# GANtastic3/MaskCycleGAN-VC

Measured on AMD Instinct MI355X. Metric: train iters/s (full G+D step), 80x64 mel bs=1, higher is better.
Workload: dtype f32

## Files before the change

include/mcvc.h:

```cpp
#ifndef MCVC_H
#define MCVC_H

#ifdef __cplusplus
extern "C" {
#endif

#define MCVC_ABI_VERSION 3
#define MCVC_GEN_NPARAMS 110
#define MCVC_DISC_NPARAMS 20
#define MCVC_N_MEL 80

int mcvc_version(void);

int mcvc_set_deterministic(int on);
int mcvc_get_deterministic(void);
int mcvc_set_precise(int on);
int mcvc_get_precise(void);
int mcvc_set_trunk_persistent(int on);

int mcvc_twin_begin(void);
int mcvc_twin_switch(void);
int mcvc_twin_end(void);
int mcvc_twin_launches(void);

// ... 155 lines not shown

int mcvc_ms_max_fft(void);
int mcvc_ms_launches(void);
int mcvc_ms_table_init(int n_fft, float* table_host);
int mcvc_ms_power(const float* cep, long long n_frames, int K, const int* offs_dev, int n_utts, const int* offs_host, int n_fft, const float* table,
                  float* power, float* mean, float* var, void* stream);
int mcvc_ms_mean_log(const float* values, int n, long long R, float floor, float* out, void* stream);
int mcvc_ms_distance(const float* a, const float* b, int K, int n_bins, int n_used, float* per_dim, float* total, void* stream);

long long mcvc_conv2d_pack_floats(int Cout, int Cin, int KH, int KW);
int mcvc_conv2d_forward(const float* x, const float* w, const float* bias, float* y, float* wpack,
                        float* slabs, int max_slabs, int N, int Cin, int H, int W, int Cout, int KH, int KW,
                        int stride, int pad_h, int pad_w, int pixel_shuffle, void* stream);
int mcvc_conv2d_dgrad(const float* dy, const float* w, float* dx, float* wpack, float* slabs, int max_slabs,
                      int N, int Cin, int H, int W, int Cout, int KH, int KW, int stride, int pad_h, int pad_w,
                      void* stream);
long long mcvc_conv2d_wgrad_slab_floats(int N, int Cin, int H, int W, int Cout, int KH, int KW, int stride, int pad_h, int pad_w);
int mcvc_conv2d_wgrad(const float* x, const float* dy, float* dw, float* slabs, long long slab_floats, int N, int Cin, int H, int W,
                      int Cout, int KH, int KW, int stride, int pad_h, int pad_w, void* stream);
long long mcvc_layer_packed_floats(int Cin, int Cout, int branches, int KH, int KW, int stride, int pad_h, int pad_w);
long long mcvc_layer_scratch_floats(int N, int H, int W, int Cin, int Cout, int branches, int KH, int KW, int stride, int pad_h, int pad_w);
int mcvc_layer_pack(const float* w0, const float* b0, const float* w1, const float* b1, float* packed, int Cin, int Cout, int branches,
                    int KH, int KW, int stride, int pad_h, int pad_w, void* stream);
int mcvc_layer_forward(const float* x, const float* packed, const float* w0, const float* w1, float* y, float* scratch,
                       long long scratch_floats, int N, int H, int W, int Cin, int Cout, int branches, int KH, int KW, int stride,
                       int pad_h, int pad_w, int scheme, int pixel_shuffle, void* stream);
int mcvc_layer_dgrad(const float* dy, const float* packed, const float* w0, const float* w1, float* dx, float* scratch,
                     long long scratch_floats, int N, int H, int W, int Cin, int Cout, int branches, int KH, int KW, int stride,
                     int pad_h, int pad_w, int scheme, void* stream);
int mcvc_layer_wgrad(const float* x, const float* dy, float* dw0, float* dw1, float* scratch, long long scratch_floats, int N, int H,
                     int W, int Cin, int Cout, int branches, int KH, int KW, int stride, int pad_h, int pad_w, int scheme, void* stream);
int mcvc_layer_wgrad_flags(const float* x, const float* dy, float* dw0, float* dw1, float* scratch, long long scratch_floats, int N, int H,
                           int W, int Cin, int Cout, int branches, int KH, int KW, int stride, int pad_h, int pad_w, int scheme, int flags,
                           void* stream);
int mcvc_trunk_layer_backward(const float* dy, const float* conv_out, const float* stats, const float* gamma, const float* beta,
                              const float* gamma_gate, const float* beta_gate, const float* w, const float* w_gate, const float* x_in,
                              float* dx, float* dconv, float* dgamma, float* dbeta, float* dgamma_gate, float* dbeta_gate, float* dw,
                              float* dw_gate, float* wpack, int B, int Cin, int T4, int Cout, int KW, void* stream);

int mcvc_instnorm_act_forward(float* x, const float* gamma, const float* beta, const float* gamma_gate,
                              const float* beta_gate, const float* residual, float* y, float* stats,
                              int N, int C, int H, int W, int act, void* stream);
int mcvc_instnorm_act_backward(const float* x, const float* gamma, const float* beta, const float* gamma_gate,
                               const float* beta_gate, const float* stats, float* dy, float* dx,
                               float* dgamma, float* dbeta, float* dgamma_gate, float* dbeta_gate,
                               int N, int C, int H, int W, int act, void* stream);

int mcvc_trunk_layer_forward(const float* x, const float* w, const float* bias, const float* gamma, const float* beta, const float* w_gate,
                             const float* bias_gate, const float* gamma_gate, const float* beta_gate, const float* residual, float* conv_out,
                             float* stats, float* y, int B, int Cin, int T4, int Cout, int KW, void* stream);

int mcvc_batched_gemm(const float* a, const float* b, float* c, int nbatch, int M, int N, int K, int lda, int ldb, int ldc,
                      long long a_stride, long long b_stride, long long c_stride, void* stream);

int mcvc_bias_grad(const float* dy, float* db, int N, int C, int P, void* stream);
int mcvc_act_forward(float* x, float* y, int N, int C, int P, int act, void* stream);
int mcvc_act_backward(const float* x, float* dy, float* dx, int N, int C, int P, int act, void* stream);
int mcvc_fif_input(const float* x, const float* mask, float* xin, int N, int P, void* stream);
int mcvc_fif_input_grad(const float* dxin, const float* mask, float* dx, int N, int P, int accumulate, void* stream);

int mcvc_trace_enable(int on);
int mcvc_trace_kinds(void);
const char* mcvc_trace_kind_name(int kind);
int mcvc_trace_collect(double* out);
int mcvc_trace_collect_raw(double* out, int max_records);

#ifdef __cplusplus
}
#endif
#endif
```

maskcyclegan-vc_amd/csrc/net.hip:

```cpp
#include "mcvc_common.h"
#include "twin.h"
#include "pack.h"
#include "packforms.h"
#include "misc.h"
#include "trunk.h"
#include "wino.h"
#include "wino4.h"
#include "sgemm.h"
#include "sampler.h"
#include "audio.h"
#include "vocoder.h"
#include "griffinlim.h"
#include "melinv.h"
#include "dtw.h"
#include "ms.h"
#include "f0.h"
#include "../../include/mcvc.h"
#include <string.h>
#include <algorithm>
#include <array>
#include <tuple>
#include <map>
#include <mutex>
#include <vector>
// ... 2723 lines not shown
    } else rc = mcvc_trunk_launch(a, ks, s);
    if (rc || !x_in || !dw) return rc;
    if (KW != 3 || !mcvc_wgrad_smallk_batch_applies(B, T4)) return MCVC_ERR_INVALID;
    SmallKJob jobs[2];
    int nj = 0;
    jobs[nj++] = SmallKJob{x_in, dconv, dw, Cin, Cout, 0, 0};
    if (glu && dw_gate) jobs[nj++] = SmallKJob{x_in, dconv + (long long)Cout * B * T4, dw_gate, Cin, Cout, 0, 0};
    return mcvc_wgrad_smallk_batch_launch(jobs, nj, B, T4, s);
}

int mcvc_instnorm_act_forward(float* x, const float* gamma, const float* beta, const float* gamma_gate, const float* beta_gate,
                              const float* residual, float* y, float* stats, int N, int C, int H, int W, int act, void* stream)
{
    Exec ex{}; ex.s = (hipStream_t)stream;
    NormP np{}; np.g[0] = gamma; np.b[0] = beta; np.g[1] = gamma_gate; np.b[1] = beta_gate;
    const int Cx = (act == ACT_GLU) ? 2 * C : C;
    norm_fwd(ex, x, (long long)Cx * H * W, (long long)H * W, 0, 1, np, stats, y, (long long)C * H * W, (long long)H * W, W, residual, N, C, H, W, act);
    return ex.err;
}

int mcvc_instnorm_act_backward(const float* x, const float* gamma, const float* beta, const float* gamma_gate, const float* beta_gate,
                               const float* stats, float* dy, float* dx, float* dgamma, float* dbeta, float* dgamma_gate, float* dbeta_gate,
                               int N, int C, int H, int W, int act, void* stream)
{
    Exec ex{}; ex.s = (hipStream_t)stream;
    NormP np{}; np.g[0] = gamma; np.b[0] = beta; np.g[1] = gamma_gate; np.b[1] = beta_gate;
    np.dg[0] = dgamma; np.db[0] = dbeta; np.dg[1] = dgamma_gate; np.db[1] = dbeta_gate;
    const int Cx = (act == ACT_GLU) ? 2 * C : C;
    norm_bwd(ex, x, (long long)Cx * H * W, (long long)H * W, np, stats, dy, (long long)C * H * W, (long long)H * W, W, 0, 1,
             dx, (long long)Cx * H * W, (long long)H * W, W, 0, N, C, H, W, act);
    return ex.err;
}

int mcvc_trunk_layer_forward(const float* x, const float* w, const float* bias, const float* gamma, const float* beta, const float* w_gate,
                             const float* bias_gate, const float* gamma_gate, const float* beta_gate, const float* residual, float* conv_out,
                             float* stats, float* y, int B, int Cin, int T4, int Cout, int KW, void* stream)
{
    if (!x || !w || !bias || !gamma || !beta || !conv_out || !stats || !y) return MCVC_ERR_INVALID;
    const int mode = w_gate ? TRUNK_IN_GLU : TRUNK_IN;
    if (!mcvc_trunk_applies(Cin, KW, Cout, B, T4, mode, 1)) return MCVC_ERR_INVALID;
    TrunkArgs a{};
    a.a0 = w; a.bias0 = bias; a.gamma0 = gamma; a.beta0 = beta;
    a.a1 = w_gate; a.bias1 = bias_gate; a.gamma1 = gamma_gate; a.beta1 = beta_gate;
    a.x = x; a.x_sc = (long long)B * T4; a.x_sb = T4;
    a.Cin = Cin; a.KW = KW; a.K = Cin * KW; a.M = Cout; a.Mtot = w_gate ? 2 * Cout : Cout; a.B = B; a.T4 = T4; a.N = B * T4;
    a.conv_out = conv_out; a.c_sc = (long long)B * T4; a.c_sb = T4;
    a.stats = stats; a.y = y; a.res = residual; a.y_sn = T4; a.y_sc = (long long)B * T4; a.eps = kInEps; a.mode = mode;
    return mcvc_trunk_launch(a, 1, (hipStream_t)stream);
}

int mcvc_batched_gemm(const float* a, const float* b, float* c, int nbatch, int M, int N, int K, int lda, int ldb, int ldc,
                      long long a_stride, long long b_stride, long long c_stride, void* stream)
{
    if (!a || !b || !c || nbatch < 1) return MCVC_ERR_INVALID;
    WinoGemmArgs ga{};
    ga.a = a; ga.a_xi = a_stride; ga.lda = lda; ga.b = b; ga.b_xi = b_stride; ga.ldb = ldb; ga.c = c; ga.c_xi = c_stride; ga.ldc = ldc;
    ga.M = M; ga.N = N; ga.K = K; ga.nxi = nbatch;
    return mcvc_wino_gemm_launch(ga, (hipStream_t)stream);
}

int mcvc_bias_grad(const float* dy, float* db, int N, int C, int P, void* stream)
{
    return mcvc_bias_grad_launch(dy, (long long)C * P, (long long)P, N, C, P, db, (hipStream_t)stream);
}

int mcvc_act_forward(float* x, float* y, int N, int C, int P, int act, void* stream)
{
    Exec ex{}; ex.s = (hipStream_t)stream;
    act_fwd(ex, x, 0, 1, y, N, C, P, act);
    return ex.err;
}

int mcvc_act_backward(const float* x, float* dy, float* dx, int N, int C, int P, int act, void* stream)
{
    Exec ex{}; ex.s = (hipStream_t)stream;
    act_bwd(ex, x, dy, 0, 1, dx, N, C, P, act);
    return ex.err;
}

int mcvc_fif_input(const float* x, const float* mask, float* xin, int N, int P, void* stream)
{
    return mcvc_prep_input_launch(x, mask, xin, N, P, (hipStream_t)stream);
}

int mcvc_fif_input_grad(const float* dxin, const float* mask, float* dx, int N, int P, int accumulate, void* stream)
{
    return mcvc_mask_grad_launch(dxin, nullptr, 0, 1, mask, dx, N, P, 2, accumulate, (hipStream_t)stream);
}

}
```

maskcyclegan-vc_amd/csrc/wino.h:

```cpp
#pragma once
#include <hip/hip_runtime.h>

struct WinoXformArgs {
    const float* x; long long x_sb, x_sc; int x_sh;
    float* v;
    int N, C, H, W;
    int TH, TW, NT;
    int NTp;
    int pad;
};

struct WinoOutArgs {
    const float* m;
    const float* bias;
    float* y; long long y_sb, y_sc; int y_sh;
    int N, Cout, OH, OW, TH, TW, NT, NTp;
    int shuffle, YH, YW;
    int accumulate;
};

int mcvc_wino_input_launch(const WinoXformArgs& a, hipStream_t s);
struct NormArgs;
bool mcvc_norm_fwd_wino_applies(const NormArgs& a, const WinoOutArgs& w, int pts);
int mcvc_norm_fwd_wino_launch(const NormArgs& a, const WinoOutArgs& w, int pts, hipStream_t s);
// ... 10 lines not shown
static __device__ __forceinline__ void wino_weight_core(const float* g, float* dst, int co, int ci, int ld, long long xi_stride, int co_off, int dgrad)
{
    float gg[5][5];
#pragma unroll
    for (int k = 0; k < 5; ++k)
#pragma unroll
        for (int l = 0; l < 5; ++l) gg[k][l] = dgrad ? g[(4 - k) * 5 + (4 - l)] : g[k * 5 + l];
    auto grow = [](const float v[5], float o[6]) {
        const float s_even = v[0] + v[2] + v[4], s_odd = v[1] + v[3];
        o[0] = 0.25f * v[0];
        o[1] = -(s_even + s_odd) * (1.0f / 6.0f);
        o[2] = -(s_even - s_odd) * (1.0f / 6.0f);
        const float e2 = v[0] * (1.0f / 24.0f) + v[2] * (1.0f / 6.0f) + v[4] * (2.0f / 3.0f);
        const float o2 = v[1] * (1.0f / 12.0f) + v[3] * (1.0f / 3.0f);
        o[3] = e2 + o2;
        o[4] = e2 - o2;
        o[5] = v[4];
    };
    float t[5][6];
#pragma unroll
    for (int k = 0; k < 5; ++k) grow(gg[k], t[k]);
    const long long row = dgrad ? (co_off + co) : ci;
    const long long col = dgrad ? ci : (co_off + co);
    float* d0 = dst + row * ld + col;
#pragma unroll
    for (int b = 0; b < 6; ++b) {
        float colv[5], o[6];
#pragma unroll
        for (int k = 0; k < 5; ++k) colv[k] = t[k][b];
        grow(colv, o);
#pragma unroll
        for (int aa = 0; aa < 6; ++aa) d0[(long long)(aa * 6 + b) * xi_stride] = o[aa];
    }
}
static __device__ __forceinline__ void wino_weight_tile(const float* w, float* dst, int Cout, int Cin, int ld, long long xi_stride, int co_off, int dgrad, int bx, int by)
{
    const int a_idx = bx * 256 + threadIdx.x;
    const int b_idx = by;
    const int co = dgrad ? b_idx : a_idx, ci = dgrad ? a_idx : b_idx;
    if (co >= Cout || ci >= Cin) return;
    wino_weight_core(w + ((long long)co * Cin + ci) * 25, dst, co, ci, ld, xi_stride, co_off, dgrad);
}


struct WinoGemmArgs {
    const float* a; long long a_xi; int lda;
    const float* b; long long b_xi; int ldb;
    float* c; long long c_xi; int ldc;
    int M, N, K;
    int nxi;
    int nt, mt;
    int mgroup;
};
int mcvc_wino_gemm_launch(const WinoGemmArgs& a, hipStream_t s);

template <int P>
static __device__ __forceinline__ void wino_g3(float v0, float v1, float v2, float* o)
{
    if constexpr (P == 4) { o[0] = v0; o[1] = 0.5f * (v0 + v1 + v2); o[2] = 0.5f * (v0 - v1 + v2); o[3] = v2; }
    else {
        const float e = v0 + v2, e2 = v0 * (1.0f / 24.0f) + v2 * (1.0f / 6.0f);
        o[0] = 0.25f * v0; o[1] = -(e + v1) * (1.0f / 6.0f); o[2] = -(e - v1) * (1.0f / 6.0f);
        o[3] = e2 + v1 * (1.0f / 12.0f); o[4] = e2 - v1 * (1.0f / 12.0f); o[5] = v2;
    }
}

template <int P>
static __device__ __forceinline__ void wino3_weight_core_p(const float* g, float* dst, int co, int ci, int ld, long long xi_stride, int co_off)
{
    float gg[5][5];
#pragma unroll
    for (int k = 0; k < 25; ++k) gg[k / 5][k % 5] = g[k];
#pragma unroll
    for (int qh = 0; qh < 2; ++qh)
#pragma unroll
        for (int qw = 0; qw < 2; ++qw) {
            float t[3][P];
#pragma unroll
            for (int u = 0; u < 3; ++u) {
                const int kh = qh ? 5 - 2 * u : 4 - 2 * u;
                float r0 = 0.f, r1 = 0.f, r2 = 0.f;
                if (kh <= 4) {
                    if (qw) { r1 = gg[kh][3]; r2 = gg[kh][1]; }
                    else { r0 = gg[kh][4]; r1 = gg[kh][2]; r2 = gg[kh][0]; }
                }
                wino_g3<P>(r0, r1, r2, t[u]);
            }
            float* d0 = dst + (long long)(co_off + co) * ld + 4 * ci + 2 * qh + qw;
#pragma unroll
            for (int b = 0; b < P; ++b) {
                float o[P];
                wino_g3<P>(t[0][b], t[1][b], t[2][b], o);
#pragma unroll
                for (int aa = 0; aa < P; ++aa) d0[(long long)(aa * P + b) * xi_stride] = o[aa];
            }
        }
}

template <int P>
static __device__ __forceinline__ void wino3_weight_tile_p(const float* w, float* dst, int Cout, int Cin, int ld, long long xi_stride, int co_off, int bx, int by)
{
    const int ci = bx * 256 + threadIdx.x, co = by;
    if (co >= Cout || ci >= Cin) return;
    wino3_weight_core_p<P>(w + ((long long)co * Cin + ci) * 25, dst, co, ci, ld, xi_stride, co_off);
}

template <int P>
// ... 48 lines not shown
```

maskcyclegan-vc_amd/csrc/wino_kernels.hip:

```cpp
#include "mcvc_common.h"
#include "trace.h"
#include "launch.h"
#include "wino.h"

namespace {

__device__ __forceinline__ void bt6(const float d[6], float o[6])
{
    o[0] = 4.f * d[0] - 5.f * d[2] + d[4];
    o[1] = -4.f * (d[1] + d[2]) + d[3] + d[4];
    o[2] = 4.f * (d[1] - d[2]) - d[3] + d[4];
    o[3] = -2.f * d[1] - d[2] + 2.f * d[3] + d[4];
    o[4] = 2.f * d[1] - d[2] - 2.f * d[3] + d[4];
    o[5] = 4.f * d[1] - 5.f * d[3] + d[5];
}

__global__ void __launch_bounds__(256) wino_input_kernel(const Twin<WinoXformArgs> tw)
{
    const WinoXformArgs a = tw.v[blockIdx.z];
    const int tile = blockIdx.x * 256 + threadIdx.x;
    const int c = blockIdx.y;
    if (tile >= a.NT) return;
    const int per = a.TH * a.TW;
    const int n = tile / per, r = tile - n * per;
// ... 417 lines not shown

__global__ void __launch_bounds__(256) wino_output_kernel(const Twin<WinoOutArgs> tw)
{
    const WinoOutArgs a = tw.v[blockIdx.z];
    const int tile = blockIdx.x * 256 + threadIdx.x;
    const int co = blockIdx.y;
    if (tile >= a.NT) return;
    const int per = a.TH * a.TW;
    const int n = tile / per, r = tile - n * per;
    const int ty = r / a.TW, tx = r - ty * a.TW;
    const float* src = a.m + (long long)co * a.NTp + tile;
    const long long xs = (long long)a.Cout * a.NTp;
    float u[2][6];
#pragma unroll
    for (int b = 0; b < 6; ++b) {
        float col[6];
#pragma unroll
        for (int aa = 0; aa < 6; ++aa) col[aa] = src[(long long)(aa * 6 + b) * xs];
        at6(col, u[0][b], u[1][b]);
    }
    const float bias = a.bias ? a.bias[co] : 0.f;
    float* yn = a.y + (long long)n * a.y_sb;
#pragma unroll
    for (int i = 0; i < 2; ++i) {
        float o0, o1;
        at6(u[i], o0, o1);
        const float ov[2] = {o0 + bias, o1 + bias};
        const int oh = 2 * ty + i;
#pragma unroll
        for (int j = 0; j < 2; ++j) {
            const int ow = 2 * tx + j;
            if (oh >= a.OH || ow >= a.OW) continue;
            long long off;
            if (a.shuffle) {
                const int yh = 2 * oh + ((co >> 1) & 1), yw = 2 * ow + (co & 1);
                if (yh >= a.YH || yw >= a.YW) continue;
                off = (long long)(co >> 2) * a.y_sc + (long long)yh * a.y_sh + yw;
            } else {
                off = (long long)co * a.y_sc + (long long)oh * a.y_sh + ow;
            }
            if (a.accumulate) yn[off] += ov[j]; else yn[off] = ov[j];
        }
    }
}


constexpr int kGK = 16;
constexpr int kGStages = 4;
#ifndef MCVC_FOLDK
#define MCVC_FOLDK 32
#endif
constexpr int kFoldK = MCVC_FOLDK;
constexpr int kGA = kGK * 128;

__device__ __forceinline__ void wg_glds16(const float* g, float* l)
{
    __builtin_amdgcn_global_load_lds((const __attribute__((address_space(1))) void*)g,
                                     (__attribute__((address_space(3))) void*)l, 16, 0, 0);
}

template <int BN>
__global__ void __launch_bounds__(256, (BN == 64 ? 3 : 4)) wino_gemm_kernel(const Twin<WinoGemmArgs> tw)
{
    const WinoGemmArgs a = tw.v[blockIdx.z];
    constexpr int kGB = kGK * BN;
    constexpr int kGStage = kGA + kGB;
    constexpr int NACC = (BN == 64) ? 2 : 1;
    extern __shared__ __attribute__((aligned(16))) float smem[];
    const int tid = threadIdx.x, lane = tid & 63;
    const int wave = __builtin_amdgcn_readfirstlane(tid >> 6);
    const int l31 = lane & 31, half = lane >> 5;
    const int wm = (BN == 64) ? (wave >> 1) : wave, wn = (BN == 64) ? (wave & 1) : 0;
    int lid;
    {
        const int total = (int)gridDim.x, linear = (int)blockIdx.x;
        const int q = total >> 3, r = total & 7, xcd = linear & 7, k = linear >> 3;
        lid = (xcd < r ? xcd * (q + 1) : r * (q + 1) + (xcd - r) * q) + k;
    }
    const int n0 = (lid % a.nt) * BN; lid /= a.nt;
    const int m0 = (lid % a.mt) * 128;
    const int xi = lid / a.mt;
    const float* A = a.a + (long long)xi * a.a_xi + m0;
    const float* B = a.b + (long long)xi * a.b_xi + n0;
    const int fa0 = wave * 64 + lane, fa1 = fa0 + 256;
    const float* a_src0 = A + (long long)(fa0 >> 5) * a.lda + 4 * (fa0 & 31);
    const float* a_src1 = A + (long long)(fa1 >> 5) * a.lda + 4 * (fa1 & 31);
    const int bw = (BN == 64) ? wave : (wave & 1);
    const int fb = bw * 64 + lane;
    constexpr int F4R = BN / 4;
    int bcol = 4 * (fb % F4R);
    if (n0 + bcol > a.ldb - 4) bcol = a.ldb - 4 - n0;
    const float* b_src = B + (long long)(fb / F4R) * a.ldb + bcol;
    const long long a_step = (long long)kGK * a.lda, b_step = (long long)kGK * a.ldb;
    auto issue = [&](int stage_k, int buf) {
        float* base = smem + buf * kGStage;
        wg_glds16(a_src0 + stage_k * a_step, base + (wave * 64) * 4);
        wg_glds16(a_src1 + stage_k * a_step, base + (wave * 64 + 256) * 4);
        wg_glds16(b_src + stage_k * b_step, base + kGA + (bw * 64) * 4);
    };
    f32x16 acc[NACC], tot[NACC];
#pragma unroll
    for (int i = 0; i < NACC; ++i)
#pragma unroll
        for (int r = 0; r < 16; ++r) { acc[i][r] = 0.f; tot[i][r] = 0.f; }
    constexpr int kFoldSt = kFoldK / kGK;
    const int nst = a.K / kGK;
// ... 126 lines not shown
    const int b_lane = SA + half * BN + wn * (32 * NBN) + l31;
    for (int st = 0; st < nst; ++st) {
        const int newer = (nst - 1 - st) < (ST - 2) ? (nst - 1 - st) : (ST - 2);
        if (newer >= 2) wait_vm<2 * ND>(); else if (newer == 1) wait_vm<ND>(); else wait_vm<0>();
        __builtin_amdgcn_s_barrier();
        if (st + ST - 1 < nst) issue(st + ST - 1, (st + ST - 1) % ST);
        if (st != 0 && (st % kFoldSt) == 0) {
#pragma unroll
            for (int i = 0; i < NACC; ++i)
#pragma unroll
                for (int r = 0; r < 16; ++r) { tot[i][r] += acc[i][r]; acc[i][r] = 0.f; }
        }
        const float* sb = smem + (st % ST) * STAGE;
        float av[NBM], bv[NBN];
#pragma unroll
        for (int i = 0; i < NBM; ++i) av[i] = sb[a_lane + 32 * i];
#pragma unroll
        for (int j = 0; j < NBN; ++j) bv[j] = sb[b_lane + 32 * j];
#pragma unroll
        for (int p = 0; p < GK / 2; ++p) {
            const int q = (p + 1 < GK / 2) ? p + 1 : p;
            float na[NBM], nb[NBN];
#pragma unroll
            for (int i = 0; i < NBM; ++i) na[i] = sb[a_lane + q * 2 * BM + 32 * i];
#pragma unroll
            for (int j = 0; j < NBN; ++j) nb[j] = sb[b_lane + q * 2 * BN + 32 * j];
#pragma unroll
            for (int i = 0; i < NBM; ++i)
#pragma unroll
                for (int j = 0; j < NBN; ++j) acc[i * NBN + j] = __builtin_amdgcn_mfma_f32_32x32x2f32(av[i], bv[j], acc[i * NBN + j], 0, 0, 0);
            __builtin_amdgcn_sched_group_barrier(0x100, NBM + NBN, 0);
            __builtin_amdgcn_sched_group_barrier(0x008, NACC, 0);
#pragma unroll
            for (int i = 0; i < NBM; ++i) av[i] = na[i];
#pragma unroll
            for (int j = 0; j < NBN; ++j) bv[j] = nb[j];
        }
    }
    const long long ldc = a.ldc;
    const int Nv = a.N;
    float* Cb = a.c + (long long)xi * a.c_xi + (long long)(m0 + wm * (32 * NBM) + 4 * half) * ldc;
#pragma unroll
    for (int j = 0; j < NBN; ++j) {
        const int n = n0 + wn * (32 * NBN) + 32 * j + l31;
        if (n >= Nv) continue;
        float* C = Cb + n;
#pragma unroll
        for (int i = 0; i < NBM; ++i)
#pragma unroll
            for (int r = 0; r < 16; ++r) C[(long long)(i * 32 + (r & 3) + 8 * (r >> 2)) * ldc] = tot[i * NBN + j][r] + acc[i * NBN + j][r];
    }
}

template <int BM, int BN, int GK, int ST>
static int gemm2_launch(WinoGemmArgs b, int nxi, hipStream_t s)
{
    if ((b.M % BM) != 0 || (b.K % GK) != 0) return MCVC_ERR_INVALID;
    b.nt = cdiv_i(b.N, BN); b.mt = b.M / BM;
    {
        static const int mgk = mcvc_knob("MCVC_GEMM_MGROUP", 8);
        static const int mgn = mcvc_knob("MCVC_GEMM_MGROUP_MINNT", 8);
        b.mgroup = (mgk > 0 && b.nt >= mgn) ? (mgk < b.mt ? mgk : b.mt) : 0;
    }
    constexpr size_t lds = (size_t)ST * (GK * BM + GK * BN) * sizeof(float);
    static bool done = false;
    if (!done) {
        hipError_t e = hipFuncSetAttribute(reinterpret_cast<const void*>(gemm2_kernel<BM, BN, GK, ST>), hipFuncAttributeMaxDynamicSharedMemorySize, 160 * 1024);
        if (e != hipSuccess) return (int)e;
        done = true;
    }
    mcvc_launch((gemm2_kernel<BM, BN, GK, ST>), dim3((unsigned)(b.nt * b.mt * nxi)), dim3(256), lds, s, b);
    return (int)hipGetLastError();
}

}

int mcvc_wino_input_launch(const WinoXformArgs& a, hipStream_t s)
{
    dim3 grid((unsigned)cdiv_i(a.NT, 256), (unsigned)a.C);
    TraceScope ts(K_ELEMENTWISE, s, 0.0, 4.0 * ((double)a.N * a.C * a.H * a.W + 36.0 * a.C * a.NT));
    mcvc_launch(wino_input_kernel, grid, dim3(256), 0, s, a);
    return (int)hipGetLastError();
}

int mcvc_wino_output_launch(const WinoOutArgs& a, hipStream_t s)
{
    dim3 grid((unsigned)cdiv_i(a.NT, 256), (unsigned)a.Cout);
    TraceScope ts(K_ELEMENTWISE, s, 0.0, 4.0 * (36.0 * a.Cout * a.NT + 4.0 * a.Cout * a.NT));
    mcvc_launch(wino_output_kernel, grid, dim3(256), 0, s, a);
    return (int)hipGetLastError();
}

int mcvc_wino_gemm_launch(const WinoGemmArgs& a, hipStream_t s)
{
    if ((a.K % kGK) != 0 || (a.M % 128) != 0 || (a.lda & 3) || (a.ldb & 3) || a.ldb < 64) return MCVC_ERR_INVALID;
    const int nxi = a.nxi > 0 ? a.nxi : 36;
    WinoGemmArgs b = a;
    static const int knob = mcvc_knob("MCVC_WINO_BN", 0);
    const int pad64 = cdiv_i(a.N, 64) * 64, pad32 = cdiv_i(a.N, 32) * 32;
    bool narrow = (pad64 * 10 > pad32 * 11) && a.N <= 512 && a.ldb >= 32;
    if (knob == 32) narrow = a.ldb >= 32; else if (knob == 64) narrow = false;
    b.mt = a.M / 128;
    TraceScope ts(K_WINO_GEMM, s, 2.0 * nxi * a.M * a.N * a.K, 4.0 * nxi * ((double)a.K * a.M + (double)a.K * a.N + (double)a.M * a.N));
#ifdef MCVC_EXPERIMENTS
    static const int cfg2 = mcvc_knob("MCVC_GEMM_CFG", 0);
    static const bool verbose = mcvc_knob_set("MCVC_GEMM_VERBOSE");
    if (verbose && mcvc_twin_phase() != 1) fprintf(stderr, "[gemm] nxi=%d M=%d N=%d K=%d lda=%d ldb=%d twin=%d\n", nxi, a.M, a.N, a.K, a.lda, a.ldb, mcvc_twin_phase() == 2);
    switch (cfg2) {
        case 1: return gemm2_launch<128, 64, 16, 4>(b, nxi, s);
        case 2: return gemm2_launch<128, 32, 16, 4>(b, nxi, s);
        case 3: return gemm2_launch<64, 64, 16, 4>(b, nxi, s);
        case 4: return gemm2_launch<128, 64, 32, 3>(b, nxi, s);
        case 5: return gemm2_launch<128, 32, 32, 3>(b, nxi, s);
        case 6: return gemm2_launch<64, 64, 32, 3>(b, nxi, s);
        case 7: return gemm2_launch<128, 64, 16, 6>(b, nxi, s);
        case 8: return gemm2_launch<128, 32, 16, 6>(b, nxi, s);
        case 9: return gemm2_launch<64, 64, 16, 6>(b, nxi, s);
        case 10: return gemm2_launch<128, 64, 32, 4>(b, nxi, s);
        case 11: return gemm2_launch<64, 64, 32, 4>(b, nxi, s);
        case 12: return gemm2_launch<128, 128, 16, 4>(b, nxi, s);
        case 13: return gemm2_launch<128, 128, 32, 3>(b, nxi, s);
        case 14: return gemm2_launch<128, 128, 16, 6>(b, nxi, s);
        case 15: return gemm2_launch<128, 128, 32, 2>(b, nxi, s);
        default: break;
    }
#else
    constexpr int cfg2 = 0;
#endif
    static const int big = mcvc_knob("MCVC_GEMM_BIG", 1);
    if (cfg2 == 0 && big && a.N >= 1280 && (a.K % 16) == 0 && (long long)cdiv_i(a.N, 128) * (a.M / 128) * nxi >= 1280)
        return gemm2_launch<128, 128, 16, 4>(b, nxi, s);
    auto rounds_cost = [&](int bm, int bn) { return (double)cdiv_i(cdiv_i(a.N, bn) * (a.M / bm) * nxi, 256) * bm * bn; };
    static const int costsel = mcvc_knob("MCVC_GEMM_COST", 1);
    if (cfg2 == 0 && a.K >= 512 && (a.K % 32) == 0 && (a.M % 64) == 0) {
        if (!(costsel && a.ldb >= 32 && rounds_cost(128, 32) < 0.94 * rounds_cost(64, 64))) return gemm2_launch<64, 64, 32, 4>(b, nxi, s);
        return gemm2_launch<128, 32, 16, 4>(b, nxi, s);
    }
    if (narrow) {
        b.nt = cdiv_i(a.N, 32);
        static bool done = false;
        if (!done) {
            hipError_t e = hipFuncSetAttribute(reinterpret_cast<const void*>(wino_gemm_kernel<32>), hipFuncAttributeMaxDynamicSharedMemorySize, 64 * 1024);
            if (e != hipSuccess) return (int)e;
            done = true;
        }
        mcvc_launch(wino_gemm_kernel<32>, dim3((unsigned)(b.nt * b.mt * nxi)), dim3(256), (size_t)kGStages * (kGA + kGK * 32) * sizeof(float), s, b);
    } else {
        b.nt = cdiv_i(a.N, 64);
        mcvc_launch(wino_gemm_kernel<64>, dim3((unsigned)(b.nt * b.mt * nxi)), dim3(256), (size_t)kGStages * (kGA + kGK * 64) * sizeof(float), s, b);
    }
    return (int)hipGetLastError();
}

int mcvc_wino_input_t_launch(const WinoXformArgs& a, hipStream_t s)
{
    return xform_t_launch<0>(a, 0, 0, 4.0 * ((double)a.N * a.C * a.H * a.W + 36.0 * a.C * a.NTp), s);
}

int mcvc_wino_dy_t_launch(const WinoXformArgs& a, hipStream_t s)
{
    return xform_t_launch<1>(a, 0, 0, 4.0 * ((double)a.N * a.C * a.H * a.W + 36.0 * a.C * a.NTp), s);
}

int mcvc_wino_dw_launch(const float* du, float* dw, int Cout, int Cin, int store, hipStream_t s)
{
    dim3 grid((unsigned)cdiv_i(Cin, 256), (unsigned)Cout);
    TraceScope ts(K_ELEMENTWISE, s, 0.0, 4.0 * (36.0 + (store ? 25.0 : 50.0)) * Cout * Cin);
    if (store) mcvc_launch(wino_dw_kernel<true>, grid, dim3(256), 0, s, WinoDwKArgs{du, dw, Cout, Cin});
    else mcvc_launch(wino_dw_kernel<false>, grid, dim3(256), 0, s, WinoDwKArgs{du, dw, Cout, Cin});
    return (int)hipGetLastError();
}

int mcvc_wino3_input_launch(const WinoXformArgs& a, hipStream_t s)
{
    dim3 grid((unsigned)cdiv_i(a.NT, 256), (unsigned)a.C);
    TraceScope ts(K_ELEMENTWISE, s, 0.0, 4.0 * ((double)a.N * a.C * a.H * a.W + 16.0 * a.C * a.NT));
    mcvc_launch(wino3_input_kernel, grid, dim3(256), 0, s, a);
    return (int)hipGetLastError();
}

int mcvc_wino3_output_launch(const WinoOutArgs& a, hipStream_t s)
{
    dim3 grid((unsigned)cdiv_i(a.NT, 256), (unsigned)a.Cout);
    TraceScope ts(K_ELEMENTWISE, s, 0.0, 4.0 * (16.0 * a.Cout * a.NT + 4.0 * a.Cout * a.NT));
    mcvc_launch(wino3_output_kernel, grid, dim3(256), 0, s, a);
    return (int)hipGetLastError();
}

int mcvc_wino3_input_phase_launch(const WinoXformArgs& a, int XH, int XW, hipStream_t s)
{
    dim3 grid((unsigned)cdiv_i(a.NT, 256), (unsigned)a.C);
    TraceScope ts(K_ELEMENTWISE, s, 0.0, 4.0 * ((double)a.N * (a.C / 4) * XH * XW + 16.0 * a.C * a.NT));
    mcvc_launch(wino3_input_phase_kernel, grid, dim3(256), 0, s, Wino3InputPhaseKArgs{a, XH, XW});
    return (int)hipGetLastError();
}

int mcvc_wino3_input_phase_t_launch(const WinoXformArgs& a, int XH, int XW, hipStream_t s)
{
    return xform_t_launch<2>(a, XH, XW, 4.0 * ((double)a.N * (a.C / 4) * XH * XW + 16.0 * a.C * a.NTp), s);
}
// ... 15 lines not shown
```

maskcyclegan-vc_amd/mask_cyclegan_vc/_hip.py:

```python
from __future__ import annotations

import ctypes
import os
from ctypes import c_double, c_float, c_int, c_longlong, c_void_p

import torch

_HERE = os.path.dirname(os.path.abspath(__file__))
LIB_PATH = os.environ.get("MCVC_LIB") or os.path.join(os.path.dirname(_HERE), "lib", "libmcvc_hip.so")

ABI_VERSION = 3
GEN_NPARAMS = 110
DISC_NPARAMS = 20
N_MEL = 80

_lib = None

_PP = ctypes.POINTER(c_void_p)

_SIGS = {
    "mcvc_version": (c_int, []),
    "mcvc_set_deterministic": (c_int, [c_int]),
    "mcvc_get_deterministic": (c_int, []),
    "mcvc_set_precise": (c_int, [c_int]),
# ... 76 lines not shown
    "mcvc_voc_launches": (c_int, []),
    "mcvc_voc_packed_floats": (c_longlong, []),
    "mcvc_voc_pack": (c_int, [_PP, c_void_p]),
    "mcvc_voc_workspace_floats": (c_longlong, [c_int, c_int]),
    "mcvc_voc_decode": (c_int, [c_void_p, c_void_p, c_void_p, c_void_p, c_longlong, c_int, c_int, c_void_p]),
    "mcvc_voc_layer_packed_floats": (c_longlong, [c_int] * 5),
    "mcvc_voc_layer_pack": (c_int, [c_int] + [c_void_p] * 5 + [c_int] * 4),
    "mcvc_voc_layer": (c_int, [c_int] + [c_void_p] * 4 + [c_int] * 8 + [c_void_p]),
    "mcvc_gl_out_samples": (c_int, [c_int]),
    "mcvc_gl_launches": (c_int, [c_int]),
    "mcvc_gl_tables_floats": (c_longlong, []),
    "mcvc_gl_tables_init": (c_int, [c_void_p, c_void_p]),
    "mcvc_gl_workspace_floats": (c_longlong, [c_int, c_int]),
    "mcvc_gl_decode": (c_int, [c_void_p, c_int, c_void_p, c_void_p, c_void_p, c_void_p, c_longlong, c_int, c_int, c_int, c_float, c_void_p]),
    "mcvc_melinv_max_iter": (c_int, []),
    "mcvc_melinv_tables_floats": (c_longlong, []),
    "mcvc_melinv_tables_init": (c_int, [c_void_p, c_void_p, c_double, c_void_p]),
    "mcvc_melinv_solve": (c_int, [c_void_p, c_void_p, c_void_p, c_int, c_int, c_int, c_void_p]),
    "mcvc_dtw_max_frames": (c_int, []),
    "mcvc_dtw_launches": (c_int, [c_int]),
    "mcvc_cep_basis_init": (c_int, [c_int, c_void_p]),
    "mcvc_cep_project": (c_int, [c_void_p, c_longlong, c_void_p, c_int, c_void_p, c_void_p]),
    "mcvc_dtw_plan": (c_int, [c_void_p, c_void_p, c_int, c_int, c_void_p, ctypes.POINTER(c_longlong), ctypes.POINTER(c_longlong)]),
    "mcvc_dtw_run": (c_int, [c_void_p, c_longlong, c_void_p, c_longlong, c_int, c_float, c_void_p, c_void_p, c_void_p, c_int, c_void_p, c_void_p,
                             c_void_p, c_void_p, c_longlong, c_void_p]),
    "mcvc_f0_max_lag": (c_int, []),
    "mcvc_f0_launches": (c_int, [c_int]),
    "mcvc_f0_track": (c_int, [c_void_p, c_longlong, c_void_p, c_int, c_int, c_int, c_float, c_void_p, c_void_p, c_void_p, c_longlong, c_void_p]),
    "mcvc_f0_stats": (c_int, [c_void_p, c_longlong, c_void_p, c_longlong, c_void_p, c_void_p, c_int, c_void_p, c_void_p, c_void_p]),
    "mcvc_ms_max_fft": (c_int, []),
    "mcvc_ms_launches": (c_int, []),
    "mcvc_ms_table_init": (c_int, [c_int, c_void_p]),
    "mcvc_ms_power": (c_int, [c_void_p, c_longlong, c_int, c_void_p, c_int, c_void_p, c_int, c_void_p, c_void_p, c_void_p, c_void_p, c_void_p]),
    "mcvc_ms_mean_log": (c_int, [c_void_p, c_int, c_longlong, c_float, c_void_p, c_void_p]),
    "mcvc_ms_distance": (c_int, [c_void_p, c_void_p, c_int, c_int, c_int, c_void_p, c_void_p, c_void_p]),
    "mcvc_axpy": (c_int, [c_void_p, c_void_p, c_float, c_longlong, c_void_p]),
    "mcvc_conv2d_pack_floats": (c_longlong, [c_int, c_int, c_int, c_int]),
    "mcvc_conv2d_forward": (c_int, [c_void_p] * 6 + [c_int] * 12 + [c_void_p]),
    "mcvc_conv2d_dgrad": (c_int, [c_void_p] * 5 + [c_int] * 11 + [c_void_p]),
    "mcvc_conv2d_wgrad_slab_floats": (c_longlong, [c_int] * 10),
    "mcvc_conv2d_wgrad": (c_int, [c_void_p] * 4 + [c_longlong] + [c_int] * 10 + [c_void_p]),
    "mcvc_layer_packed_floats": (c_longlong, [c_int] * 8),
    "mcvc_layer_scratch_floats": (c_longlong, [c_int] * 11),
    "mcvc_layer_pack": (c_int, [c_void_p] * 5 + [c_int] * 8 + [c_void_p]),
    "mcvc_layer_forward": (c_int, [c_void_p] * 6 + [c_longlong] + [c_int] * 13 + [c_void_p]),
    "mcvc_layer_dgrad": (c_int, [c_void_p] * 6 + [c_longlong] + [c_int] * 12 + [c_void_p]),
    "mcvc_layer_wgrad": (c_int, [c_void_p] * 5 + [c_longlong] + [c_int] * 12 + [c_void_p]),
    "mcvc_layer_wgrad_flags": (c_int, [c_void_p] * 5 + [c_longlong] + [c_int] * 13 + [c_void_p]),
    "mcvc_trunk_layer_backward": (c_int, [c_void_p] * 19 + [c_int] * 5 + [c_void_p]),
    "mcvc_instnorm_act_forward": (c_int, [c_void_p] * 8 + [c_int] * 5 + [c_void_p]),
    "mcvc_instnorm_act_backward": (c_int, [c_void_p] * 12 + [c_int] * 5 + [c_void_p]),
    "mcvc_trunk_layer_forward": (c_int, [c_void_p] * 13 + [c_int] * 5 + [c_void_p]),
    "mcvc_batched_gemm": (c_int, [c_void_p] * 3 + [c_int] * 7 + [c_longlong] * 3 + [c_void_p]),
    "mcvc_bias_grad": (c_int, [c_void_p, c_void_p, c_int, c_int, c_int, c_void_p]),
    "mcvc_act_forward": (c_int, [c_void_p, c_void_p, c_int, c_int, c_int, c_int, c_void_p]),
    "mcvc_act_backward": (c_int, [c_void_p, c_void_p, c_void_p, c_int, c_int, c_int, c_int, c_void_p]),
    "mcvc_fif_input": (c_int, [c_void_p, c_void_p, c_void_p, c_int, c_int, c_void_p]),
    "mcvc_fif_input_grad": (c_int, [c_void_p, c_void_p, c_void_p, c_int, c_int, c_int, c_void_p]),
    "mcvc_trace_enable": (c_int, [c_int]),
    "mcvc_trace_kinds": (c_int, []),
    "mcvc_trace_kind_name": (ctypes.c_char_p, [c_int]),
    "mcvc_trace_collect": (c_int, [ctypes.POINTER(ctypes.c_double)]),
    "mcvc_trace_collect_raw": (c_int, [ctypes.POINTER(ctypes.c_double), c_int]),
}

EXPORTED_SYMBOLS = tuple(_SIGS)


def lib():
    global _lib
    if _lib is None:
        if not os.path.exists(LIB_PATH):
            raise RuntimeError(
                "libmcvc_hip.so not found at %s -- build it with `python -c 'import __graft_entry__ as g; g.build()'` "
                "(hipcc --offload-arch=gfx950). There is no CPU fallback." % LIB_PATH)
        L = ctypes.CDLL(LIB_PATH)
        for name, (res, args) in _SIGS.items():
            fn = getattr(L, name)
            fn.restype = res
            fn.argtypes = args
        if L.mcvc_version() != ABI_VERSION:
            raise RuntimeError("libmcvc_hip.so ABI version mismatch")
        _lib = L
    return _lib


class twin(object):

    def __enter__(self):
        check(lib().mcvc_twin_begin(), "mcvc_twin_begin")
        return self

    def switch(self):
        check(lib().mcvc_twin_switch(), "mcvc_twin_switch")

    def __exit__(self, et, ev, tb):
        rc = lib().mcvc_twin_end()
        if et is None:
            check(rc, "mcvc_twin_end (the two call sequences of a grouped pass differ)")
        return False


def check(rc: int, what: str = "mcvc call"):
    if rc != 0:
        raise RuntimeError("%s failed with code %d" % (what, rc))

# ... 55 lines not shown
```

Before: 183.9.

## Add persistent tile-looping GEMM variant with planner and use 3 stages for 64x64

Adds a persistent version of the batched Winograd GEMM kernel. It launches at most occupancy-times-CU blocks, and each block walks a contiguous range of tiles, spread evenly across the XCDs. The goal is to cut tail-wave waste and per-block launch overhead when there are more tiles than resident slots. The tile-shape choice moves into a separate plan function, which now uses the real CU count and an optional tie-break. New ABI entry points expose flags, the plan and the slot count. The persistent path is off by default through a compile-time knob, but the 64x64 config now defaults to 3 pipeline stages instead of 4, which uses less LDS per block at the cost of less latency hiding.

```diff
diff --git a/include/mcvc.h b/include/mcvc.h
--- a/include/mcvc.h
+++ b/include/mcvc.h
@@ -231,6 +231,10 @@
 
 int mcvc_batched_gemm(const float* a, const float* b, float* c, int nbatch, int M, int N, int K, int lda, int ldb, int ldc,
                       long long a_stride, long long b_stride, long long c_stride, void* stream);
+int mcvc_batched_gemm_flags(const float* a, const float* b, float* c, int nbatch, int M, int N, int K, int lda, int ldb, int ldc,
+                            long long a_stride, long long b_stride, long long c_stride, void* stream, int flags);
+int mcvc_batched_gemm_plan(int nbatch, int M, int N, int K, int lda, int ldb, int flags);
+int mcvc_batched_gemm_slots(int tile_rows, int tile_cols);
 
 int mcvc_bias_grad(const float* dy, float* db, int N, int C, int P, void* stream);
 int mcvc_act_forward(float* x, float* y, int N, int C, int P, int act, void* stream);
diff --git a/maskcyclegan-vc_amd/csrc/net.hip b/maskcyclegan-vc_amd/csrc/net.hip
--- a/maskcyclegan-vc_amd/csrc/net.hip
+++ b/maskcyclegan-vc_amd/csrc/net.hip
@@ -2799,11 +2799,27 @@
 int mcvc_batched_gemm(const float* a, const float* b, float* c, int nbatch, int M, int N, int K, int lda, int ldb, int ldc,
                       long long a_stride, long long b_stride, long long c_stride, void* stream)
 {
-    if (!a || !b || !c || nbatch < 1) return MCVC_ERR_INVALID;
+    return mcvc_batched_gemm_flags(a, b, c, nbatch, M, N, K, lda, ldb, ldc, a_stride, b_stride, c_stride, stream, 0);
+}
+
+int mcvc_batched_gemm_flags(const float* a, const float* b, float* c, int nbatch, int M, int N, int K, int lda, int ldb, int ldc,
+                            long long a_stride, long long b_stride, long long c_stride, void* stream, int flags)
+{
+    if (!a || !b || !c || nbatch < 1 || (flags & ~3) || (flags & 3) == 3) return MCVC_ERR_INVALID;
     WinoGemmArgs ga{};
     ga.a = a; ga.a_xi = a_stride; ga.lda = lda; ga.b = b; ga.b_xi = b_stride; ga.ldb = ldb; ga.c = c; ga.c_xi = c_stride; ga.ldc = ldc;
     ga.M = M; ga.N = N; ga.K = K; ga.nxi = nbatch;
-    return mcvc_wino_gemm_launch(ga, (hipStream_t)stream);
+    return mcvc_wino_gemm_launch(ga, (hipStream_t)stream, flags);
+}
+
+int mcvc_batched_gemm_slots(int tile_rows, int tile_cols) { return mcvc_wino_gemm_slots(tile_rows, tile_cols); }
+
+int mcvc_batched_gemm_plan(int nbatch, int M, int N, int K, int lda, int ldb, int flags)
+{
+    if (nbatch < 1 || (flags & ~3) || (flags & 3) == 3) return MCVC_ERR_INVALID;
+    WinoGemmArgs ga{};
+    ga.lda = lda; ga.ldb = ldb; ga.M = M; ga.N = N; ga.K = K; ga.nxi = nbatch;
+    return mcvc_wino_gemm_plan(ga, flags);
 }
 
 int mcvc_bias_grad(const float* dy, float* db, int N, int C, int P, void* stream)
diff --git a/maskcyclegan-vc_amd/csrc/wino.h b/maskcyclegan-vc_amd/csrc/wino.h
--- a/maskcyclegan-vc_amd/csrc/wino.h
+++ b/maskcyclegan-vc_amd/csrc/wino.h
@@ -86,7 +86,9 @@
     int nt, mt;
     int mgroup;
 };
-int mcvc_wino_gemm_launch(const WinoGemmArgs& a, hipStream_t s);
+int mcvc_wino_gemm_launch(const WinoGemmArgs& a, hipStream_t s, int flags = 0);
+int mcvc_wino_gemm_plan(const WinoGemmArgs& a, int flags);
+int mcvc_wino_gemm_slots(int bm, int bn);
 
 template <int P>
 static __device__ __forceinline__ void wino_g3(float v0, float v1, float v2, float* o)
diff --git a/maskcyclegan-vc_amd/csrc/wino_kernels.hip b/maskcyclegan-vc_amd/csrc/wino_kernels.hip
--- a/maskcyclegan-vc_amd/csrc/wino_kernels.hip
+++ b/maskcyclegan-vc_amd/csrc/wino_kernels.hip
@@ -493,6 +493,12 @@
 #endif
 constexpr int kFoldK = MCVC_FOLDK;
 constexpr int kGA = kGK * 128;
+#ifndef MCVC_GEMM_PERSIST_DEFAULT
+#define MCVC_GEMM_PERSIST_DEFAULT 0
+#endif
+#ifndef MCVC_GEMM_TIEPAD_DEFAULT
+#define MCVC_GEMM_TIEPAD_DEFAULT 0
+#endif
 
 __device__ __forceinline__ void wg_glds16(const float* g, float* l)
 {
@@ -725,6 +731,169 @@
     }
 }
 
+struct TileCur { int xi, g, gm, n_t, mi; };
+__device__ __forceinline__ void tile_decode(TileCur& c, int lid, int mt, int nt, int mg)
+{
+    const int per = mt * nt;
+    int r = lid % per;
+    c.xi = lid / per;
+    c.g = r / (mg * nt);
+    c.gm = (c.g + 1) * mg <= mt ? mg : mt - c.g * mg;
+    r -= c.g * mg * nt;
+    c.n_t = r / c.gm; c.mi = r % c.gm;
+}
+__device__ __forceinline__ void tile_next(TileCur& c, int mt, int nt, int mg)
+{
+    if (++c.mi < c.gm) return;
+    c.mi = 0;
+    if (++c.n_t < nt) return;
+    c.n_t = 0;
+    if (++c.g * mg >= mt) { c.g = 0; ++c.xi; }
+    c.gm = (c.g + 1) * mg <= mt ? mg : mt - c.g * mg;
+}
+
+template <int BM, int BN, int GK, int ST>
+__global__ void __launch_bounds__(256) gemm2_persist_kernel(const Twin<WinoGemmArgs> tw)
+{
+    const WinoGemmArgs a = tw.v[blockIdx.z];
+    constexpr int SA = GK * BM, SB = GK * BN, STAGE = SA + SB;
+    constexpr bool W22 = (BN % 64) == 0;
+    constexpr int NBM = W22 ? BM / 64 : BM / 128, NBN = W22 ? BN / 64 : BN / 32, NACC = NBM * NBN;
+    constexpr int NA = (SA / 4 + 255) / 256, NB = (SB / 4 + 255) / 256, ND = NA + NB;
+    static_assert(2 * ND <= 63, "vmcnt immediate");
+    extern __shared__ __attribute__((aligned(16))) float smem[];
+    const int tid = threadIdx.x, lane = tid & 63;
+    const int wave = __builtin_amdgcn_readfirstlane(tid >> 6);
+    const int l31 = lane & 31, half = lane >> 5;
+    const int wm = W22 ? (wave >> 1) : wave, wn = W22 ? (wave & 1) : 0;
+    const int mt = a.mt, nt = a.nt, mg = a.mgroup > 0 ? a.mgroup : 1;
+    int first, cnt;
+    {
+        const int total = (int)gridDim.x, linear = (int)blockIdx.x;
+        const int q8 = total >> 3, r8 = total & 7, xcd = linear & 7, k = linear >> 3;
+        const int p = (xcd < r8 ? xcd * (q8 + 1) : r8 * (q8 + 1) + (xcd - r8) * q8) + k;
+        const long long tiles = (long long)mt * nt * a.nxi;
+        first = (int)(p * tiles / total);
+        cnt = (int)((p + 1) * tiles / total) - first;
+    }
+    TileCur ic, cc;
+    tile_decode(ic, first, mt, nt, mg);
+    cc = ic;
+    constexpr int A4R = BM / 4, B4R = BN / 4;
+    const int lda = a.lda, ldb = a.ldb;
+    int aoff[NA], adst[NA], brow[NB], bcl[NB], bdst[NB];
+#pragma unroll
+    for (int i = 0; i < NA; ++i) {
+        const int f = (tid + i * 256) % (SA / 4);
+        aoff[i] = (f / A4R) * lda + 4 * (f % A4R);
+        adst[i] = (((wave * 64 + i * 256) % (SA / 4))) * 4;
+    }
+#pragma unroll
+    for (int i = 0; i < NB; ++i) {
+        const int f = (tid + i * 256) % (SB / 4);
+        brow[i] = (f / B4R) * ldb; bcl[i] = 4 * (f % B4R);
+        bdst[i] = SA + (((wave * 64 + i * 256) % (SB / 4))) * 4;
+    }
+    const long long a_step = (long long)GK * lda, b_step = (long long)GK * ldb;
+    const int nst = a.K / GK;
+    const int S = cnt * nst;
+    const float* ia; const float* ib; int boff[NB];
+    auto issue_tile = [&]() {
+        const int m0 = (ic.g * mg + ic.mi) * BM, n0 = ic.n_t * BN;
+        ia = a.a + (long long)ic.xi * a.a_xi + m0;
+        ib = a.b + (long long)ic.xi * a.b_xi + n0;
+#pragma unroll
+        for (int i = 0; i < NB; ++i) {
+            int bcol = bcl[i];
+            if (n0 + bcol > ldb - 4) bcol = ldb - 4 - n0;
+            boff[i] = brow[i] + bcol;
+        }
+    };
+    int ig = 0, ik = 0;
+    auto issue_next = [&]() {
+        float* base = smem + (ig % ST) * STAGE;
+#pragma unroll
+        for (int i = 0; i < NA; ++i) wg_glds16(ia + aoff[i], base + adst[i]);
+#pragma unroll
+        for (int i = 0; i < NB; ++i) wg_glds16(ib + boff[i], base + bdst[i]);
+        ++ig;
+        if (++ik < nst) { ia += a_step; ib += b_step; }
+        else { ik = 0; tile_next(ic, mt, nt, mg); if (ig < S) issue_tile(); }
+    };
+    issue_tile();
+#pragma unroll
+    for (int s = 0; s < ST - 1; ++s)
+        if (ig < S) issue_next();
+    f32x16 acc[NACC], tot[NACC];
+#pragma unroll
+    for (int i = 0; i < NACC; ++i)
+#pragma unroll
+        for (int r = 0; r < 16; ++r) { acc[i][r] = 0.f; tot[i][r] = 0.f; }
+    constexpr int kFoldSt = kFoldK / GK;
+    const int a_lane = half * BM + wm * (32 * NBM) + l31;
+    const int b_lane = SA + half * BN + wn * (32 * NBN) + l31;
+    const long long ldc = a.ldc;
+    const int Nv = a.N;
+    int g = 0;
+    for (int t = 0; t < cnt; ++t) {
+        for (int st = 0; st < nst; ++st, ++g) {
+            const int rem = S - 1 - g, newer = rem < (ST - 2) ? rem : (ST - 2);
+            if (newer >= 2) wait_vm<2 * ND>(); else if (newer == 1) wait_vm<ND>(); else wait_vm<0>();
+            __builtin_amdgcn_s_barrier();
+            if (ig < S) issue_next();
+            if (st != 0 && (st % kFoldSt) == 0) {
+#pragma unroll
+                for (int i = 0; i < NACC; ++i)
+#pragma unroll
+                    for (int r = 0; r < 16; ++r) { tot[i][r] += acc[i][r]; acc[i][r] = 0.f; }
+            }
+            const float* sb = smem + (g % ST) * STAGE;
+            float av[NBM], bv[NBN];
+#pragma unroll
+            for (int i = 0; i < NBM; ++i) av[i] = sb[a_lane + 32 * i];
+#pragma unroll
+            for (int j = 0; j < NBN; ++j) bv[j] = sb[b_lane + 32 * j];
+#pragma unroll
+            for (int p = 0; p < GK / 2; ++p) {
+                const int q = (p + 1 < GK / 2) ? p + 1 : p;
+                float na[NBM], nb[NBN];
+#pragma unroll
+                for (int i = 0; i < NBM; ++i) na[i] = sb[a_lane + q * 2 * BM + 32 * i];
+#pragma unroll
+                for (int j = 0; j < NBN; ++j) nb[j] = sb[b_lane + q * 2 * BN + 32 * j];
+#pragma unroll
+                for (int i = 0; i < NBM; ++i)
+#pragma unroll
+                    for (int j = 0; j < NBN; ++j) acc[i * NBN + j] = __builtin_amdgcn_mfma_f32_32x32x2f32(av[i], bv[j], acc[i * NBN + j], 0, 0, 0);
+                __builtin_amdgcn_sched_group_barrier(0x100, NBM + NBN, 0);
+                __builtin_amdgcn_sched_group_barrier(0x008, NACC, 0);
+#pragma unroll
+                for (int i = 0; i < NBM; ++i) av[i] = na[i];
+#pragma unroll
+                for (int j = 0; j < NBN; ++j) bv[j] = nb[j];
+            }
+        }
+        const int m0 = (cc.g * mg + cc.mi) * BM, n0 = cc.n_t * BN;
+        float* Cb = a.c + (long long)cc.xi * a.c_xi + (long long)(m0 + wm * (32 * NBM) + 4 * half) * ldc;
+#pragma unroll
+        for (int j = 0; j < NBN; ++j) {
+            const int n = n0 + wn * (32 * NBN) + 32 * j + l31;
+            if (n < Nv) {
+                float* C = Cb + n;
+#pragma unroll
+                for (int i = 0; i < NBM; ++i)
+#pragma unroll
+                    for (int r = 0; r < 16; ++r) C[(long long)(i * 32 + (r & 3) + 8 * (r >> 2)) * ldc] = tot[i * NBN + j][r] + acc[i * NBN + j][r];
+            }
+#pragma unroll
+            for (int i = 0; i < NBM; ++i)
+#pragma unroll
+                for (int r = 0; r < 16; ++r) { acc[i * NBN + j][r] = 0.f; tot[i * NBN + j][r] = 0.f; }
+        }
+        tile_next(cc, mt, nt, mg);
+    }
+}
+
 template <int BM, int BN, int GK, int ST>
 static int gemm2_launch(WinoGemmArgs b, int nxi, hipStream_t s)
 {
@@ -746,6 +915,43 @@
     return (int)hipGetLastError();
 }
 
+template <int BM, int BN, int GK, int ST>
+static int gemm2_persist_slots(int* cus)
+{
+    static int slots = 0, ncu = 0;
+    if (slots == 0) {
+        constexpr size_t lds = (size_t)ST * (GK * BM + GK * BN) * sizeof(float);
+        const void* fn = reinterpret_cast<const void*>(gemm2_persist_kernel<BM, BN, GK, ST>);
+        int dev = 0, occ = 0;
+        slots = -1;
+        if (hipFuncSetAttribute(fn, hipFuncAttributeMaxDynamicSharedMemorySize, 160 * 1024) == hipSuccess && hipGetDevice(&dev) == hipSuccess &&
+            hipDeviceGetAttribute(&ncu, hipDeviceAttributeMultiprocessorCount, dev) == hipSuccess &&
+            hipOccupancyMaxActiveBlocksPerMultiprocessor(&occ, gemm2_persist_kernel<BM, BN, GK, ST>, 256, lds) == hipSuccess && occ > 0 && ncu > 0)
+            slots = occ * ncu;
+    }
+    if (cus) *cus = ncu;
+    return slots;
+}
+
+template <int BM, int BN, int GK, int ST>
+static int gemm2_persist_launch(WinoGemmArgs b, int nxi, hipStream_t s)
+{
+    if ((b.M % BM) != 0 || (b.K % GK) != 0 || b.K < GK) return MCVC_ERR_INVALID;
+    b.nt = cdiv_i(b.N, BN); b.mt = b.M / BM; b.nxi = nxi;
+    {
+        static const int mgk = mcvc_knob("MCVC_GEMM_MGROUP", 8);
+        static const int mgn = mcvc_knob("MCVC_GEMM_MGROUP_MINNT", 8);
+        b.mgroup = (mgk > 0 && b.nt >= mgn) ? (mgk < b.mt ? mgk : b.mt) : 0;
+    }
+    constexpr size_t lds = (size_t)ST * (GK * BM + GK * BN) * sizeof(float);
+    int slots = gemm2_persist_slots<BM, BN, GK, ST>(nullptr);
+    if (slots <= 0) return MCVC_ERR_INVALID;
+    if (mcvc_twin_phase() != 0) slots = slots > 1 ? slots / 2 : 1;
+    const long long tiles = (long long)b.nt * b.mt * nxi;
+    mcvc_launch((gemm2_persist_kernel<BM, BN, GK, ST>), dim3((unsigned)(tiles < slots ? tiles : slots)), dim3(256), lds, s, b);
+    return (int)hipGetLastError();
+}
+
 }
 
 int mcvc_wino_input_launch(const WinoXformArgs& a, hipStream_t s)
@@ -764,15 +970,66 @@
     return (int)hipGetLastError();
 }
 
-int mcvc_wino_gemm_launch(const WinoGemmArgs& a, hipStream_t s)
+template <int BM, int BN, int GK, int ST>
+static bool gemm2_use_persist(const WinoGemmArgs& b, int nxi, int persist)
+{
+    if (b.K < GK || persist == 0) return false;
+    if (persist > 0) return true;
+    int slots = gemm2_persist_slots<BM, BN, GK, ST>(nullptr);
+    if (mcvc_twin_phase() != 0) slots /= 2;
+    return slots > 0 && (long long)cdiv_i(b.N, BN) * (b.M / BM) * nxi > slots;
+}
+template <int BM, int BN, int GK, int ST>
+static int gemm2_either(const WinoGemmArgs& b, int nxi, int persist, hipStream_t s)
+{
+    return gemm2_use_persist<BM, BN, GK, ST>(b, nxi, persist) ? gemm2_persist_launch<BM, BN, GK, ST>(b, nxi, s) : gemm2_launch<BM, BN, GK, ST>(b, nxi, s);
+}
+
+int mcvc_wino_gemm_slots(int bm, int bn)
+{
+    if (bm == 64 && bn == 64) return gemm2_persist_slots<64, 64, 32, 3>(nullptr);
+    if (bm == 128 && bn == 32) return gemm2_persist_slots<128, 32, 16, 4>(nullptr);
+    if (bm == 128 && bn == 64) return gemm2_persist_slots<128, 64, 16, 4>(nullptr);
+    if (bm == 128 && bn == 128) return gemm2_persist_slots<128, 128, 16, 4>(nullptr);
+    return MCVC_ERR_INVALID;
+}
+
+int mcvc_wino_gemm_plan(const WinoGemmArgs& a, int flags)
 {
     if ((a.K % kGK) != 0 || (a.M % 128) != 0 || (a.lda & 3) || (a.ldb & 3) || a.ldb < 64) return MCVC_ERR_INVALID;
-    const int nxi = a.nxi > 0 ? a.nxi : 36;
-    WinoGemmArgs b = a;
+    const int nxi = (a.nxi > 0 ? a.nxi : 36);
     static const int knob = mcvc_knob("MCVC_WINO_BN", 0);
     const int pad64 = cdiv_i(a.N, 64) * 64, pad32 = cdiv_i(a.N, 32) * 32;
     bool narrow = (pad64 * 10 > pad32 * 11) && a.N <= 512 && a.ldb >= 32;
     if (knob == 32) narrow = a.ldb >= 32; else if (knob == 64) narrow = false;
+    int bm, bn;
+    static const int big = mcvc_knob("MCVC_GEMM_BIG", 1);
+    static const int costsel = mcvc_knob("MCVC_GEMM_COST", 1);
+    static const int tiepad = mcvc_knob("MCVC_GEMM_TIEPAD", MCVC_GEMM_TIEPAD_DEFAULT);
+    int cus = 0;
+    if (gemm2_persist_slots<64, 64, 32, 3>(&cus) <= 0 || cus <= 0) cus = 256;
+    auto rounds_cost = [&](int rm, int rn) { return (double)cdiv_i(cdiv_i(a.N, rn) * (a.M / rm) * nxi, cus) * rm * rn; };
+    if (big && a.N >= 1280 && (a.K % 16) == 0 && (long long)cdiv_i(a.N, 128) * (a.M / 128) * nxi >= 1280) { bm = 128; bn = 128; }
+    else if (a.K >= 512 && (a.K % 32) == 0 && (a.M % 64) == 0) {
+        const double c32 = rounds_cost(128, 32), c64 = rounds_cost(64, 64);
+        const bool tie = tiepad > 0 && c32 == c64 && pad64 * 100 >= pad32 * (100 + tiepad);
+        if (costsel && a.ldb >= 32 && (c32 < 0.94 * c64 || tie)) { bm = 128; bn = 32; } else { bm = 64; bn = 64; }
+    }
+    else { bm = 128; bn = narrow ? 32 : 64; }
+    static const int pdef = mcvc_knob("MCVC_GEMM_PERSIST", MCVC_GEMM_PERSIST_DEFAULT);
+    const int form = (bm == 64) ? 1 : (bn == 32) ? 2 : (bn == 128) ? 4 : 8;
+    const int persist = (flags & 1) ? 0 : (flags & 2) ? 1 : (pdef & form) ? -1 : 0;
+    return (bm << 16) | (bn << 4) | (persist & 3);
+}
+
+int mcvc_wino_gemm_launch(const WinoGemmArgs& a, hipStream_t s, int flags)
+{
+    if ((a.K % kGK) != 0 || (a.M % 128) != 0 || (a.lda & 3) || (a.ldb & 3) || a.ldb < 64) return MCVC_ERR_INVALID;
+    const int nxi = a.nxi > 0 ? a.nxi : 36;
+    WinoGemmArgs b = a;
+    const int plan = mcvc_wino_gemm_plan(a, flags);
+    if (plan < 0) return plan;
+    const int bm = plan >> 16, bn = (plan >> 4) & 0xfff, persist = (plan & 3) == 3 ? -1 : (plan & 3);
     b.mt = a.M / 128;
     TraceScope ts(K_WINO_GEMM, s, 2.0 * nxi * a.M * a.N * a.K, 4.0 * nxi * ((double)a.K * a.M + (double)a.K * a.N + (double)a.M * a.N));
 #ifdef MCVC_EXPERIMENTS
@@ -800,16 +1057,13 @@
 #else
     constexpr int cfg2 = 0;
 #endif
-    static const int big = mcvc_knob("MCVC_GEMM_BIG", 1);
-    if (cfg2 == 0 && big && a.N >= 1280 && (a.K % 16) == 0 && (long long)cdiv_i(a.N, 128) * (a.M / 128) * nxi >= 1280)
-        return gemm2_launch<128, 128, 16, 4>(b, nxi, s);
-    auto rounds_cost = [&](int bm, int bn) { return (double)cdiv_i(cdiv_i(a.N, bn) * (a.M / bm) * nxi, 256) * bm * bn; };
-    static const int costsel = mcvc_knob("MCVC_GEMM_COST", 1);
-    if (cfg2 == 0 && a.K >= 512 && (a.K % 32) == 0 && (a.M % 64) == 0) {
-        if (!(costsel && a.ldb >= 32 && rounds_cost(128, 32) < 0.94 * rounds_cost(64, 64))) return gemm2_launch<64, 64, 32, 4>(b, nxi, s);
-        return gemm2_launch<128, 32, 16, 4>(b, nxi, s);
-    }
-    if (narrow) {
+    (void)cfg2;
+    if (bm == 128 && bn == 128) return gemm2_either<128, 128, 16, 4>(b, nxi, persist, s);
+    static const int st64 = mcvc_knob("MCVC_GEMM_ST64", 3);
+    if (bm == 64) return st64 == 3 ? gemm2_either<64, 64, 32, 3>(b, nxi, persist, s) : gemm2_either<64, 64, 32, 4>(b, nxi, persist, s);
+    if (bn == 32 && a.K >= 512) return gemm2_either<128, 32, 16, 4>(b, nxi, persist, s);
+    if (bn == 32) {
+        if (gemm2_use_persist<128, 32, 16, 4>(b, nxi, persist)) return gemm2_persist_launch<128, 32, 16, 4>(b, nxi, s);
         b.nt = cdiv_i(a.N, 32);
         static bool done = false;
         if (!done) {
@@ -819,6 +1073,7 @@
         }
         mcvc_launch(wino_gemm_kernel<32>, dim3((unsigned)(b.nt * b.mt * nxi)), dim3(256), (size_t)kGStages * (kGA + kGK * 32) * sizeof(float), s, b);
     } else {
+        if (gemm2_use_persist<128, 64, 16, 4>(b, nxi, persist)) return gemm2_persist_launch<128, 64, 16, 4>(b, nxi, s);
         b.nt = cdiv_i(a.N, 64);
         mcvc_launch(wino_gemm_kernel<64>, dim3((unsigned)(b.nt * b.mt * nxi)), dim3(256), (size_t)kGStages * (kGA + kGK * 64) * sizeof(float), s, b);
     }
diff --git a/maskcyclegan-vc_amd/mask_cyclegan_vc/_hip.py b/maskcyclegan-vc_amd/mask_cyclegan_vc/_hip.py
--- a/maskcyclegan-vc_amd/mask_cyclegan_vc/_hip.py
+++ b/maskcyclegan-vc_amd/mask_cyclegan_vc/_hip.py
@@ -152,6 +152,9 @@
     "mcvc_instnorm_act_backward": (c_int, [c_void_p] * 12 + [c_int] * 5 + [c_void_p]),
     "mcvc_trunk_layer_forward": (c_int, [c_void_p] * 13 + [c_int] * 5 + [c_void_p]),
     "mcvc_batched_gemm": (c_int, [c_void_p] * 3 + [c_int] * 7 + [c_longlong] * 3 + [c_void_p]),
+    "mcvc_batched_gemm_flags": (c_int, [c_void_p] * 3 + [c_int] * 7 + [c_longlong] * 3 + [c_void_p, c_int]),
+    "mcvc_batched_gemm_plan": (c_int, [c_int] * 7),
+    "mcvc_batched_gemm_slots": (c_int, [c_int] * 2),
     "mcvc_bias_grad": (c_int, [c_void_p, c_void_p, c_int, c_int, c_int, c_void_p]),
     "mcvc_act_forward": (c_int, [c_void_p, c_void_p, c_int, c_int, c_int, c_int, c_void_p]),
     "mcvc_act_backward": (c_int, [c_void_p, c_void_p, c_void_p, c_int, c_int, c_int, c_int, c_void_p]),
```

New measurement: 183.6. About the same (-0.1%).
